# vLAR-group/NVFi

Hardware: AMD Instinct MI355X
Metric: training rays/sec (fwd+bwd incl. PDE loss), 'bat' scene (higher is better)
Workload: dtype f32; 1 GPU; bat.yaml + velocity field + PDE divergence loss (configs[2]): 199^3 grid, K=16, 128 samples/ray, 2 renders x 2048 rays + PDE on 262144 collocation points + plane regularisers + Adam, per GPU; pde_points_per_gpu=262144, samples_per_ray=128, parallelism=ray-sharded x1, driver=fused, launch=eager launches, field=stationary (optimiser steps a shadow copy)

## Files before the change

nvfi_amd/csrc/vel_x6w.hip:

```cpp
#include <stdlib.h>
#include <utility>
#include "common.h"
#include "vel.h"
#include "pde.h"
#include "engine16.h"
#include "x6.h"

typedef unsigned u32x4w __attribute__((ext_vector_type(4)));
typedef const b8_t __attribute__((address_space(1))) * x6w_gptr;
#define X6W_ENTRIES 136
#define X6W_RING 8
#define X6W_OB_H8 (8 * 3 * 64)
#define X6W_LDS_BYTES ((6 * 128 + 4 * 2 * 16 * 8) * 4 + 4 * X6W_OB_H8 * 16)

#ifdef X6W_TIMING
__device__ unsigned long long x6w_ts[32];
#define X6W_STAMP(c, k) do { if ((c).stamp) x6w_ts[k] = __builtin_amdgcn_s_memtime(); } while (0)
#else
#define X6W_STAMP(c, k) do { } while (0)
#endif
#if defined(X6W_BUFLD)
typedef unsigned u32x4b __attribute__((ext_vector_type(4)));
#define X6W_OPAQUE(c) asm volatile("" : "+s"((c).so))
#define X6W_LD(c, P, E) __builtin_bit_cast(b8_t, __builtin_amdgcn_raw_buffer_load_b128((c).R##P, (int)(c).vo + (E) * 1024, (c).so, 0))
#define X6W_PTR(img, lane) ((x6w_gptr)(img))
#else
#define X6W_OPAQUE(c) asm volatile("" : "+v"((c).W1), "+v"((c).W2), "+v"((c).W3))
#define X6W_LD(c, P, E) ((c).P[(E) * 64])
#define X6W_PTR(img, lane) ((x6w_gptr)((img) + (lane)))
#endif
struct X6W {
    int stamp;
    unsigned vo;
#ifdef X6W_BUFLD
    __amdgpu_buffer_rsrc_t RW1, RW2, RW3; int so;
#endif
    x6w_gptr W1, W2, W3;
    const float* lb;
    const float4* w5l;
    b8_t* ob;
    float* zp;
    int lane, h;
};

template <int... Is, class F> __device__ __forceinline__ void x6w_for(std::integer_sequence<int, Is...>, F f) { (f(std::integral_constant<int, Is>{}), ...); }

struct X6WEpi {
    float rr[16];
    unsigned pk[3][8];
    float p[6];
    float4 wa, wb;
    float out[6];
    float* zst;
};
__device__ __forceinline__ float x6w_add_halves(float p) {
    const auto r = __builtin_amdgcn_permlane32_swap(__float_as_uint(p), __float_as_uint(p), false, false);
    return __uint_as_float(r[0]) + __uint_as_float(r[1]);
}
template <int U, bool LAST, int STASH = 0, bool PX4 = false>
__device__ __forceinline__ void x6w_micro(const X6W& c, float (&v)[16], X6WEpi& e, int m2) {
    if constexpr (STASH && U < 32 && (U & 1) == 0) {
        if constexpr (PX4) {
            if constexpr ((U & 7) == 0) {
                const f32x4s q = {v[U >> 1], v[(U >> 1) + 1], v[(U >> 1) + 2], v[(U >> 1) + 3]};
                __builtin_nontemporal_store(q, reinterpret_cast<f32x4s*>(e.zst - c.lane) + c.lane + (U >> 3) * 64);
            }
        } else STASH_ST(e.zst[(U >> 1) * REGF], v[U >> 1]);
    }
#ifndef X6W_PROBE_NO_SILU
    if constexpr (U < 32) {
        constexpr int r = U >> 1;
        if constexpr ((U & 1) == 0) e.rr[r] = __builtin_amdgcn_exp2f(-1.44269504088896341f * v[r]);
        else e.rr[r] = __builtin_amdgcn_rcpf(1.f + e.rr[r]);
    }
    if constexpr (U >= 2 && U <= 32 && (U & 1) == 0) { constexpr int r = (U - 2) >> 1; v[r] = v[r] * e.rr[r]; }
#endif
    if constexpr (LAST) {
        const float4* wl = c.w5l + ((m2 >> 1) * 2 + c.h) * 32;
        if constexpr (U == 0) {
#pragma unroll
            for (int o = 0; o < 6; ++o) e.p[o] = 0.f;
        }
        if constexpr (U == 1) e.wa = wl[0];
        if constexpr (U == 2) e.wb = wl[1];
        x6w_for(std::make_integer_sequence<int, 48>{}, [&](auto Gc) {
            constexpr int g = decltype(Gc)::value, r = g / 3, j = g % 3;
            if constexpr (3 + g - g / 8 == U) {
                if constexpr (j == 0) { e.p[0] = __builtin_fmaf(v[r], e.wa.x, e.p[0]); e.p[1] = __builtin_fmaf(v[r], e.wa.y, e.p[1]); }
                if constexpr (j == 1) {
                    e.p[2] = __builtin_fmaf(v[r], e.wa.z, e.p[2]); e.p[3] = __builtin_fmaf(v[r], e.wa.w, e.p[3]);
                    if constexpr (r < 15) e.wa = wl[2 * (r + 1)];
                }
                if constexpr (j == 2) {
                    e.p[4] = __builtin_fmaf(v[r], e.wb.x, e.p[4]); e.p[5] = __builtin_fmaf(v[r], e.wb.y, e.p[5]);
                    if constexpr (r < 15) e.wb = wl[2 * (r + 1) + 1];
                }
            }
        });
        if constexpr (U == 46) {
#pragma unroll
            for (int o = 0; o < 3; ++o) e.p[o] = x6w_add_halves(e.p[o]);
        }
        if constexpr (U == 47) {
#pragma unroll
            for (int o = 3; o < 6; ++o) e.p[o] = x6w_add_halves(e.p[o]);
#pragma unroll
            for (int o = 0; o < 6; ++o) e.out[o] += e.p[o];
        }
    } else {
        if constexpr (U >= 5 && U <= 36) {
            constexpr int p = (U - 5) >> 2, part = (U - 5) & 3;
#ifdef X6W_PROBE_NO_SPLIT
            if constexpr (part == 0) {
                e.pk[0][p] = __builtin_amdgcn_perm(__float_as_uint(v[2 * p + 1]), __float_as_uint(v[2 * p]), 0x07060302u);
                e.pk[1][p] = e.pk[0][p]; e.pk[2][p] = e.pk[0][p];
            }
#else
            if constexpr (part == 0) {
                const unsigned ua = __float_as_uint(v[2 * p]), ub = __float_as_uint(v[2 * p + 1]);
                e.pk[0][p] = __builtin_amdgcn_perm(ub, ua, 0x07060302u);
                e.rr[2 * p] = v[2 * p] - __uint_as_float(ua & 0xffff0000u);
            } else if constexpr (part == 1) {
                e.rr[2 * p + 1] = v[2 * p + 1] - __uint_as_float(__float_as_uint(v[2 * p + 1]) & 0xffff0000u);
            } else if constexpr (part == 2) {
                const unsigned va = __float_as_uint(e.rr[2 * p]), vb = __float_as_uint(e.rr[2 * p + 1]);
                e.pk[1][p] = __builtin_amdgcn_perm(vb, va, 0x07060302u);
                e.rr[2 * p] = e.rr[2 * p] - __uint_as_float(va & 0xffff0000u);
            } else {
                const float sb = e.rr[2 * p + 1] - __uint_as_float(__float_as_uint(e.rr[2 * p + 1]) & 0xffff0000u);
                e.pk[2][p] = __builtin_amdgcn_perm(__float_as_uint(sb), __float_as_uint(e.rr[2 * p]), 0x07060302u);
            }
#endif
        }
        if constexpr (U == 22 || U == 37) {
            constexpr int k = U == 22 ? 0 : 1;
#pragma unroll
            for (int term = 0; term < 3; ++term) {
                const u32x4w q = {e.pk[term][4 * k], e.pk[term][4 * k + 1], e.pk[term][4 * k + 2], e.pk[term][4 * k + 3]};
                c.ob[((size_t)(m2 + k) * 3 + term) * 64] = __builtin_bit_cast(b8_t, q);
            }
        }
    }
}
template <int U0, int N, bool LAST, int STASH = 0, bool PX4 = false>
__device__ __forceinline__ void x6w_micros(const X6W& c, float (&v)[16], X6WEpi& e, int m2) {
    x6w_for(std::make_integer_sequence<int, N>{}, [&](auto Uc) {
        constexpr int U = U0 + decltype(Uc)::value;
        if constexpr (U < (LAST ? 48 : 38)) x6w_micro<U, LAST, STASH, PX4>(c, v, e, m2);
    });
}
__device__ __forceinline__ void x6w_load_in(const X6W& c, b8_t (&in)[8][3], int s) {
    in[s][0] = c.ob[((size_t)s * 3 + 0) * 64]; in[s][1] = c.ob[((size_t)s * 3 + 1) * 64]; in[s][2] = c.ob[((size_t)s * 3 + 2) * 64];
}

template <int J, bool FIRST>
__device__ __forceinline__ void x6w_mfma(const b8_t& A1, const b8_t& A2, const b8_t& A3, const b8_t (&B)[3], f32x16& a0, f32x16& a1) {
    const f32x16 zero = {0.f, 0.f, 0.f, 0.f, 0.f, 0.f, 0.f, 0.f, 0.f, 0.f, 0.f, 0.f, 0.f, 0.f, 0.f, 0.f};
    if constexpr (J == 0) a0 = MFMA16B(A1, B[0], a0);
    else if constexpr (J == 1) a1 = MFMA16B(A1, B[1], FIRST ? zero : a1);
    else if constexpr (J == 2) a1 = MFMA16B(A2, B[1], a1);
    else if constexpr (J == 3) a1 = MFMA16B(A2, B[0], a1);
    else if constexpr (J == 4) a1 = MFMA16B(A1, B[2], a1);
    else a1 = MFMA16B(A3, B[0], a1);
}

template <int E0, int KIND, int LROW, bool HAVE_PE, bool PE_LAST, int STASH = 0>
__device__ __forceinline__ void x6w_tile(X6W& c, b8_t (&A1)[X6W_RING], b8_t (&A2)[X6W_RING], b8_t (&A3)[X6W_RING], const b8_t (&X0)[2][3], b8_t (&in)[8][3],
                                         float (&pv)[16], X6WEpi& e, int pm2, float (&nv)[16], f32x16& bias) {
    constexpr int NS = KIND == 0 ? 2 : 8;
    f32x16 a0 = bias, a1;
    x6w_for(std::make_integer_sequence<int, NS * 6>{}, [&](auto Ic) {
        constexpr int I = decltype(Ic)::value, s = I / 6, j = I % 6, en = E0 + s;
        if constexpr (KIND == 0) x6w_mfma<j, s == 0>(A1[en % X6W_RING], A2[en % X6W_RING], A3[en % X6W_RING], X0[s], a0, a1);
        else x6w_mfma<j, s == 0>(A1[en % X6W_RING], A2[en % X6W_RING], A3[en % X6W_RING], in[s], a0, a1);
        __builtin_amdgcn_sched_barrier(0);
        if constexpr (j == 5 && en + X6W_RING - 1 < X6W_ENTRIES + X6W_RING - 1) {
            constexpr int x = en + X6W_RING - 1;
            if constexpr ((x & 3) == 0) {
#ifndef X6W_PROBE_SAME_ENTRIES
#ifdef X6W_BUFLD
                c.so += (x == X6W_ENTRIES) ? -(X6W_ENTRIES / 4 - 1) * 4096 : 4096;
#else
                constexpr int adv = (x == X6W_ENTRIES) ? -(X6W_ENTRIES / 4 - 1) * 256 : 256;
                c.W1 += adv; c.W2 += adv; c.W3 += adv;
#endif
#endif
                X6W_OPAQUE(c);
            }
#if defined(X6W_PROBE_QUARTER_LOADS)
            if constexpr ((x & 3) == 0) { A1[x % X6W_RING] = X6W_LD(c, W1, 0); A2[x % X6W_RING] = X6W_LD(c, W2, 0); A3[x % X6W_RING] = X6W_LD(c, W3, 0); }
#elif defined(X6W_PROBE_LDS_A)
            A1[x % X6W_RING] = c.ob[((x & 7) * 3 + 0) * 64]; A2[x % X6W_RING] = c.ob[((x & 7) * 3 + 1) * 64]; A3[x % X6W_RING] = c.ob[((x & 7) * 3 + 2) * 64];
#else
            A1[x % X6W_RING] = X6W_LD(c, W1, x & 3); A2[x % X6W_RING] = X6W_LD(c, W2, x & 3); A3[x % X6W_RING] = X6W_LD(c, W3, x & 3);
#endif
        }
#ifndef X6W_PROBE_NO_EPILOGUE
        if constexpr (HAVE_PE) {
            if constexpr (KIND == 0) {
                if constexpr (I < 2) x6w_micros<4 * I, 4, PE_LAST, STASH, (STASH == 2 && LROW >= 32 && LROW - 32 < 512)>(c, pv, e, pm2);
                else x6w_micros<8 + 3 * (I - 2), 3, PE_LAST, STASH, (STASH == 2 && LROW >= 32 && LROW - 32 < 512)>(c, pv, e, pm2);
            } else if constexpr (KIND == 1) {
                if constexpr (I < 8) x6w_micros<2 * I, 2, PE_LAST, STASH, (STASH == 2 && LROW >= 32 && LROW - 32 < 512)>(c, pv, e, pm2);
                else if constexpr (I < 30) x6w_micros<I + 8, 1, PE_LAST, STASH, (STASH == 2 && LROW >= 32 && LROW - 32 < 512)>(c, pv, e, pm2);
            } else if constexpr (I < (PE_LAST ? 48 : 38)) x6w_micros<I, 1, PE_LAST, STASH, (STASH == 2 && LROW >= 32 && LROW - 32 < 512)>(c, pv, e, pm2);
        }
#endif
        if constexpr (KIND == 1 && I == 30) { x6w_load_in(c, in, 6); x6w_load_in(c, in, 7); }
        if constexpr (I == 1 && LROW + 32 < 640) {
#pragma unroll
            for (int r = 0; r < 16; ++r) bias[r] = c.lb[LROW + 32 + (r & 3) + 8 * (r >> 2) + 4 * c.h];
        }
        if constexpr (KIND == 3) {
            if constexpr (j == 5 && s < 4) x6w_load_in(c, in, s);
            if constexpr (I == 40) { x6w_load_in(c, in, 4); x6w_load_in(c, in, 5); }
        }
        __builtin_amdgcn_sched_barrier(0);
    });
#pragma unroll
    for (int r = 0; r < 16; ++r) nv[r] = a1[r] + a0[r];
    if constexpr (STASH) {
        if constexpr (KIND == 4) {
#pragma unroll
            for (int r = 0; r < 16; ++r) STASH_ST(c.zp[r * REGF], nv[r]);
        } else e.zst = c.zp;
        c.zp += 16 * REGF;
        asm volatile("" : "+v"(c.zp));
    }
    X6W_STAMP(c, E0 < 8 ? 1 + E0 / 2 : 5 + (E0 - 8) / 8);
    __builtin_amdgcn_sched_barrier(0);
}

struct X6WRing { b8_t A1[X6W_RING], A2[X6W_RING], A3[X6W_RING]; };
__device__ __forceinline__ void x6w_prime(const X6W& c0, X6WRing& R) {
    X6W c = c0;
    X6W_OPAQUE(c);
#pragma unroll
    for (int en = 0; en < X6W_RING - 1; ++en) {
#ifdef X6W_BUFLD
        if (en == 4) c.so += 4096;
#else
        if (en == 4) { c.W1 += 256; c.W2 += 256; c.W3 += 256; }
#endif
        R.A1[en] = X6W_LD(c, W1, en & 3); R.A2[en] = X6W_LD(c, W2, en & 3); R.A3[en] = X6W_LD(c, W3, en & 3);
    }
}
template <int STASH = 0>
__device__ __forceinline__ void velnet_x6w(const X6W& c0, X6WRing& R, const float4& q, float (&out6)[6], float* zst = nullptr, float* x0st = nullptr) {
    X6W c = c0;
    X6W_STAMP(c, 0);
    c.zp = STASH ? zst + c0.lane : nullptr;
    X6W_OPAQUE(c);
    b8_t X0[2][3], in[8][3];
    b8_t (&A1)[X6W_RING] = R.A1, (&A2)[X6W_RING] = R.A2, (&A3)[X6W_RING] = R.A3;
    X6WEpi e;
    float va[16], vb[16];
    {
        float x0[16];
#ifdef X6W_PROBE_NO_ENC
#pragma unroll
        for (int k = 0; k < 16; ++k) x0[k] = q.x + (float)k * q.y;
#else
        vel_encode_slots(q, c.h, x0);
#endif
        if (STASH) stash_store<16>(x0st, c.lane, x0);
#pragma unroll
        for (int k = 0; k < 2; ++k) {
            unsigned p1[4], p2[4], p3[4];
#pragma unroll
            for (int j = 0; j < 4; ++j) {
                const float xa = x0[8 * k + 2 * j], xb = x0[8 * k + 2 * j + 1];
                const unsigned ua = __float_as_uint(xa), ub = __float_as_uint(xb);
                p1[j] = __builtin_amdgcn_perm(ub, ua, 0x07060302u);
                const float ra = xa - __uint_as_float(ua & 0xffff0000u), rb = xb - __uint_as_float(ub & 0xffff0000u);
                const unsigned wa = __float_as_uint(ra), wb = __float_as_uint(rb);
                p2[j] = __builtin_amdgcn_perm(wb, wa, 0x07060302u);
                const float sa = ra - __uint_as_float(wa & 0xffff0000u), sb = rb - __uint_as_float(wb & 0xffff0000u);
                p3[j] = __builtin_amdgcn_perm(__float_as_uint(sb), __float_as_uint(sa), 0x07060302u);
            }
            const u32x4w q1 = {p1[0], p1[1], p1[2], p1[3]}, q2 = {p2[0], p2[1], p2[2], p2[3]}, q3 = {p3[0], p3[1], p3[2], p3[3]};
            X0[k][0] = __builtin_bit_cast(b8_t, q1); X0[k][1] = __builtin_bit_cast(b8_t, q2); X0[k][2] = __builtin_bit_cast(b8_t, q3);
        }
    }
#ifdef X6W_BUFLD
    c.so += 4096;
#else
    c.W1 += 256; c.W2 += 256; c.W3 += 256;
#endif
    f32x16 bias;
#pragma unroll
    for (int r = 0; r < 16; ++r) bias[r] = c.lb[(r & 3) + 8 * (r >> 2) + 4 * c.h];
#pragma unroll
    for (int o = 0; o < 6; ++o) e.out[o] = c.lb[128 * 5 + o];
    x6w_tile<0, 0, 0, false, false, STASH>(c, A1, A2, A3, X0, in, va, e, 0, va, bias);
    x6w_tile<2, 0, 32, true, false, STASH>(c, A1, A2, A3, X0, in, va, e, 0, vb, bias);
    x6w_tile<4, 0, 64, true, false, STASH>(c, A1, A2, A3, X0, in, vb, e, 2, va, bias);
    x6w_tile<6, 0, 96, true, false, STASH>(c, A1, A2, A3, X0, in, va, e, 4, vb, bias);
#pragma unroll
    for (int s = 0; s < 6; ++s) x6w_load_in(c, in, s);
    x6w_tile<8, 1, 128, true, false, STASH>(c, A1, A2, A3, X0, in, vb, e, 6, va, bias);
    x6w_tile<16, 2, 160, true, false, STASH>(c, A1, A2, A3, X0, in, va, e, 0, vb, bias);
    x6w_tile<24, 2, 192, true, false, STASH>(c, A1, A2, A3, X0, in, vb, e, 2, va, bias);
    x6w_tile<32, 3, 224, true, false, STASH>(c, A1, A2, A3, X0, in, va, e, 4, vb, bias);
    x6w_tile<40, 1, 256, true, false, STASH>(c, A1, A2, A3, X0, in, vb, e, 6, va, bias);
    x6w_tile<48, 2, 288, true, false, STASH>(c, A1, A2, A3, X0, in, va, e, 0, vb, bias);
    x6w_tile<56, 2, 320, true, false, STASH>(c, A1, A2, A3, X0, in, vb, e, 2, va, bias);
    x6w_tile<64, 3, 352, true, false, STASH>(c, A1, A2, A3, X0, in, va, e, 4, vb, bias);
    x6w_tile<72, 1, 384, true, false, STASH>(c, A1, A2, A3, X0, in, vb, e, 6, va, bias);
    x6w_tile<80, 2, 416, true, false, STASH>(c, A1, A2, A3, X0, in, va, e, 0, vb, bias);
    x6w_tile<88, 2, 448, true, false, STASH>(c, A1, A2, A3, X0, in, vb, e, 2, va, bias);
    x6w_tile<96, 3, 480, true, false, STASH>(c, A1, A2, A3, X0, in, va, e, 4, vb, bias);
    x6w_tile<104, 1, 512, true, false, STASH>(c, A1, A2, A3, X0, in, vb, e, 6, va, bias);
    x6w_tile<112, 2, 544, true, true, STASH>(c, A1, A2, A3, X0, in, va, e, 0, vb, bias);
    x6w_tile<120, 2, 576, true, true, STASH>(c, A1, A2, A3, X0, in, vb, e, 2, va, bias);
    x6w_tile<128, 4, 608, true, true, STASH>(c, A1, A2, A3, X0, in, va, e, 4, vb, bias);
#ifdef X6W_PROBE_NO_OUT
#pragma unroll
    for (int o = 0; o < 6; ++o) out6[o] = e.out[o];
    out6[0] += vb[0]; out6[1] += vb[5];
    return;
#endif
    {
        float p[6] = {0.f, 0.f, 0.f, 0.f, 0.f, 0.f};
        const float4* wl = c.w5l + (3 * 2 + c.h) * 32;
#pragma unroll
        for (int r = 0; r < 16; ++r) {
            const float4 wa = wl[2 * r], wb = wl[2 * r + 1];
            const float av = act_f<1>(vb[r]);
            p[0] = __builtin_fmaf(av, wa.x, p[0]); p[1] = __builtin_fmaf(av, wa.y, p[1]); p[2] = __builtin_fmaf(av, wa.z, p[2]);
            p[3] = __builtin_fmaf(av, wa.w, p[3]); p[4] = __builtin_fmaf(av, wb.x, p[4]); p[5] = __builtin_fmaf(av, wb.y, p[5]);
        }
#pragma unroll
        for (int o = 0; o < 6; ++o) out6[o] = e.out[o] + x6w_add_halves(p[o]);
    }
    X6W_STAMP(c, 21);
}

__global__ __launch_bounds__(WG_THREADS, 1) void k_rk2_x6w(X6Args a) {
    extern __shared__ __attribute__((aligned(16))) float lds[];
    float* lb = lds;
    float* w5f = lb + 6 * 128;
    b8_t* obase = reinterpret_cast<b8_t*>(w5f + 4 * 2 * 16 * 8);
    const int lane = threadIdx.x & 63, h = lane >> 5;
    const int wv = __builtin_amdgcn_readfirstlane(threadIdx.x >> 6);
    const int count = a.count ? *a.count : (int)a.n_direct;
    if ((int)blockIdx.x * 4 * TILE >= count) return;
    for (int k = threadIdx.x; k < 6 * 128; k += WG_THREADS) lb[k] = (k & 127) < (k < 640 ? 128 : 6) ? a.f.vb[k >> 7][k & 127] : 0.f;
    for (int k = threadIdx.x; k < 4 * 2 * 16 * 8; k += WG_THREADS) {
        const int o = k & 7, r = (k >> 3) & 15, hh = (k >> 7) & 1, ww = k >> 8;
        w5f[k] = o < 6 ? a.f.vW[5][o * 128 + 32 * ww + (r & 3) + 8 * (r >> 2) + 4 * hh] : 0.f;
    }
    __syncthreads();
    const int tile = blockIdx.x * 4 + wv;
    if (tile * TILE >= count) return;
    const int i = tile * TILE + (lane & 31);
    const bool active = i < count;
    const int n = active ? (a.list ? a.list[i] : i) : 0;
    const float4 q0 = active ? a.xw[n] : zero4();
    float x = q0.x, y = q0.y, z = q0.z;
    const float zw = q0.w;
    const int ti = a.pt_by_list ? n : i;
    float tcur = active ? a.pt_t[ti] : 0.f;
    float off = active ? tcur - a.pt_base[ti] : 0.f;
    X6W c; c.stamp = 0;
    const b8_t* img = reinterpret_cast<const b8_t*>(a.img);
    c.W1 = X6W_PTR(img, lane); c.W2 = X6W_PTR(img + X6_H8, lane); c.W3 = X6W_PTR(img + 2 * X6_H8, lane); c.vo = (unsigned)lane * 16u;
#ifdef X6W_BUFLD
    c.so = 0;
    c.RW1 = __builtin_amdgcn_make_buffer_rsrc(const_cast<b8_t*>(img), 0, 0x7fffffff, 0x00020000);
    c.RW2 = __builtin_amdgcn_make_buffer_rsrc(const_cast<b8_t*>(img + X6_H8), 0, 0x7fffffff, 0x00020000);
    c.RW3 = __builtin_amdgcn_make_buffer_rsrc(const_cast<b8_t*>(img + 2 * X6_H8), 0, 0x7fffffff, 0x00020000);
#endif
    c.lb = lb; c.w5l = reinterpret_cast<const float4*>(w5f); c.ob = obase + (size_t)wv * X6W_OB_H8 + lane; c.lane = lane; c.h = h;
    X6WRing ring;
    x6w_prime(c, ring);
#pragma unroll 1
    for (int s = 0; s < a.max_steps; ++s) {
        const bool live = active && fabsf(off) > 0.f;
        const float dt = rk2_point_dt(off, a.dt_max);
        if (!__any(live)) break;
        const float hdt = 0.5f * dt;
        float px = x, py = y, pz = z;
        float o6[6];
#pragma unroll 1
        for (int ev = 0; ev < 2; ++ev) {
            const float4 q = make_float4(px, py, pz, ev ? tcur - hdt : tcur);
#ifdef X6W_TIMING
            c.stamp = (blockIdx.x == 700 && wv == 1 && s == 2 && ev == 0) ? 1 : 0;
#endif
            velnet_x6w(c, ring, q, o6);
            if (ev == 0) {
                float v1[3];
                vel_from_w(o6, x, y, z, v1);
                if (gated_out(a.f, x, y, z)) { v1[0] = v1[1] = v1[2] = 0.f; }
                px = x - hdt * v1[0]; py = y - hdt * v1[1]; pz = z - hdt * v1[2];
            }
        }
        float v2[3];
        vel_from_w(o6, px, py, pz, v2);
        if (gated_out(a.f, px, py, pz)) { v2[0] = v2[1] = v2[2] = 0.f; }
        const float nx = x - dt * v2[0], ny = y - dt * v2[1], nz = z - dt * v2[2];
        const bool rej = a.f.gate_sur && gated_out(a.f, nx, ny, nz);
        if (live && !rej) { x = nx; y = ny; z = nz; }
        if (live) { off = off - dt; tcur = tcur - dt; }
    }
#ifdef X6W_TIMING
    if (blockIdx.x == 700 && wv == 1 && lane == 0) {
        printf("[x6w timing] tiles (layer 0: 4, layers 1-4: 4 each), then the last row tile's sums:");
        for (int k = 1; k <= 21; ++k) printf(" %llu", x6w_ts[k] - x6w_ts[k - 1]);
        printf(" | total %llu\n", x6w_ts[21] - x6w_ts[0]);
    }
#endif
    if (active && h == 0) {
        if (a.xout3) { float* o = a.xout3 + 3 * (size_t)n; o[0] = x; o[1] = y; o[2] = z; }
        else a.xw[n] = make_float4(x, y, z, zw);
    }
}

template <int STASH>
__global__ __launch_bounds__(WG_THREADS, 1) void k_rk2_x6w_uni(X6UniArgs a) {
    extern __shared__ __attribute__((aligned(16))) float lds[];
    float* lb = lds;
    float* w5f = lb + 6 * 128;
    b8_t* obase = reinterpret_cast<b8_t*>(w5f + 4 * 2 * 16 * 8);
    const Rk2Args& ra = a.r;
    const int lane = threadIdx.x & 63, h = lane >> 5;
    const int wv = __builtin_amdgcn_readfirstlane(threadIdx.x >> 6);
    const int count = *ra.count;
    if ((int)blockIdx.x * WG_SAMPLES >= count) return;
    for (int k = threadIdx.x; k < 6 * 128; k += WG_THREADS) lb[k] = (k & 127) < (k < 640 ? 128 : 6) ? ra.f.vb[k >> 7][k & 127] : 0.f;
    for (int k = threadIdx.x; k < 4 * 2 * 16 * 8; k += WG_THREADS) {
        const int o = k & 7, r = (k >> 3) & 15, hh = (k >> 7) & 1, ww = k >> 8;
        w5f[k] = o < 6 ? ra.f.vW[5][o * 128 + 32 * ww + (r & 3) + 8 * (r >> 2) + 4 * hh] : 0.f;
    }
    __syncthreads();
    const size_t tile = (size_t)blockIdx.x * 4 + wv;
    if (!STASH && (int)(tile * TILE) >= count) return;
    const int idx = (int)tile * TILE + (lane & 31);
    const bool active = idx < count;
    const int n = active ? ra.list[idx] : 0;
    const float4 q0 = active ? ra.xw[n] : zero4();
    float x = q0.x, y = q0.y, z = q0.z;
    const float zw = q0.w;
    X6W c; c.stamp = 0;
    const b8_t* img = reinterpret_cast<const b8_t*>(a.img);
    c.W1 = X6W_PTR(img, lane); c.W2 = X6W_PTR(img + X6_H8, lane); c.W3 = X6W_PTR(img + 2 * X6_H8, lane); c.vo = (unsigned)lane * 16u;
#ifdef X6W_BUFLD
    c.so = 0;
    c.RW1 = __builtin_amdgcn_make_buffer_rsrc(const_cast<b8_t*>(img), 0, 0x7fffffff, 0x00020000);
    c.RW2 = __builtin_amdgcn_make_buffer_rsrc(const_cast<b8_t*>(img + X6_H8), 0, 0x7fffffff, 0x00020000);
    c.RW3 = __builtin_amdgcn_make_buffer_rsrc(const_cast<b8_t*>(img + 2 * X6_H8), 0, 0x7fffffff, 0x00020000);
#endif
    c.lb = lb; c.w5l = reinterpret_cast<const float4*>(w5f); c.ob = obase + (size_t)wv * X6W_OB_H8 + lane; c.lane = lane; c.h = h; c.zp = nullptr;
    const int nsteps = ra.sched ? __float_as_int(ra.sched[2]) : ra.nsteps;
    X6WRing ring;
    x6w_prime(c, ring);
#pragma unroll 1
    for (int s = 0; s < nsteps; ++s) {
        const float dt = RK_DT(ra, s), tcur = RK_TC(ra, s), hdt = 0.5f * dt;
        float px = x, py = y, pz = z;
        float o6[6], w1[6];
        bool g1 = false;
#pragma unroll 1
        for (int ev = 0; ev < 2; ++ev) {
            const size_t e = (size_t)(2 * s + ev) * ra.cap_tiles + tile;
            const float4 q = make_float4(px, py, pz, ev ? tcur - hdt : tcur);
            velnet_x6w<STASH>(c, ring, q, o6, STASH ? ra.zst + e * (VEL_Z_REGS * REGF) : nullptr, STASH ? ra.x0st + e * (VEL_X0_REGS * REGF) : nullptr);
            if (ev == 0) {
                float v1[3];
#pragma unroll
                for (int k = 0; k < 6; ++k) w1[k] = o6[k];
                vel_from_w(w1, x, y, z, v1);
                g1 = gated_out(ra.f, x, y, z);
                if (g1) { v1[0] = v1[1] = v1[2] = 0.f; }
                px = x - hdt * v1[0]; py = y - hdt * v1[1]; pz = z - hdt * v1[2];
            }
        }
        float v2[3];
        vel_from_w(o6, px, py, pz, v2);
        const bool g2 = gated_out(ra.f, px, py, pz);
        if (g2) { v2[0] = v2[1] = v2[2] = 0.f; }
        const float nx = x - dt * v2[0], ny = y - dt * v2[1], nz = z - dt * v2[2];
        const bool rej = ra.f.gate_sur && gated_out(ra.f, nx, ny, nz);
        if (STASH && active && h == 0) {
            float* rc = ra.rec + (size_t)s * RK_NF * ra.cap + idx;
            rc[0 * ra.cap] = x; rc[1 * ra.cap] = y; rc[2 * ra.cap] = z;
            rc[3 * ra.cap] = px; rc[4 * ra.cap] = py; rc[5 * ra.cap] = pz;
#pragma unroll
            for (int k = 0; k < 6; ++k) { rc[(6 + k) * ra.cap] = w1[k]; rc[(12 + k) * ra.cap] = o6[k]; }
            rc[18 * ra.cap] = __int_as_float((g1 ? 1 : 0) | (g2 ? 2 : 0) | (rej ? 4 : 0));
        }
        if (active && !rej) { x = nx; y = ny; z = nz; }
    }
    if (active && h == 0) ra.xw[n] = make_float4(x, y, z, zw);
}

int launch_rk2_x6w_uni(const X6UniArgs& a, int64_t cap_samples, bool stash, hipStream_t st) {
    const int64_t groups = (cap_samples + WG_SAMPLES - 1) / WG_SAMPLES;
    if (groups <= 0) return 0;
    static DeviceOnce once;
    if (once.lds(X6W_LDS_BYTES, k_rk2_x6w_uni<2>, k_rk2_x6w_uni<1>, k_rk2_x6w_uni<0>)) return 1;
    if (stash && a.r.z_x4) hipLaunchKernelGGL(k_rk2_x6w_uni<2>, dim3((unsigned)groups), dim3(WG_THREADS), X6W_LDS_BYTES, st, a);
    else if (stash) hipLaunchKernelGGL(k_rk2_x6w_uni<1>, dim3((unsigned)groups), dim3(WG_THREADS), X6W_LDS_BYTES, st, a);
    else hipLaunchKernelGGL(k_rk2_x6w_uni<0>, dim3((unsigned)groups), dim3(WG_THREADS), X6W_LDS_BYTES, st, a);
    LAUNCHCK();
    return 0;
}

int launch_rk2_x6w(const X6Args& a, int64_t cap_points, hipStream_t st) {
    const int64_t tiles = (cap_points + TILE - 1) / TILE;
    if (tiles <= 0) return 0;
    static DeviceOnce once;
    if (once.lds(X6W_LDS_BYTES, k_rk2_x6w)) return 1;
    hipLaunchKernelGGL(k_rk2_x6w, dim3((unsigned)((tiles + 3) / 4)), dim3(WG_THREADS), X6W_LDS_BYTES, st, a);
    LAUNCHCK();
    return 0;
}
```

Measured before the change: 1.105 million rays/s.

## Process two point tiles per wave in RK2 velocity MLP to share weight loads

Adds a new RK2 kernel in which each wave advects two 32-point tiles at once. It interleaves their MFMA chains so that each weight fragment loaded from global memory is reused for both tiles. The weight ring is shortened to 4 entries and the LDS staging buffer is split per tile to make room for the doubled activation state. The new kernel is the default unless the switch selects the old path. It raises register pressure and halves the number of waves covering the points, which can hurt latency hiding. The shared LDS staging and context setup are factored into helpers.

```diff
diff --git a/nvfi_amd/csrc/vel_x6w.hip b/nvfi_amd/csrc/vel_x6w.hip
--- a/nvfi_amd/csrc/vel_x6w.hip
+++ b/nvfi_amd/csrc/vel_x6w.hip
@@ -336,23 +336,28 @@
     X6W_STAMP(c, 21);
 }
 
-__global__ __launch_bounds__(WG_THREADS, 1) void k_rk2_x6w(X6Args a) {
-    extern __shared__ __attribute__((aligned(16))) float lds[];
-    float* lb = lds;
-    float* w5f = lb + 6 * 128;
-    b8_t* obase = reinterpret_cast<b8_t*>(w5f + 4 * 2 * 16 * 8);
-    const int lane = threadIdx.x & 63, h = lane >> 5;
-    const int wv = __builtin_amdgcn_readfirstlane(threadIdx.x >> 6);
-    const int count = a.count ? *a.count : (int)a.n_direct;
-    if ((int)blockIdx.x * 4 * TILE >= count) return;
-    for (int k = threadIdx.x; k < 6 * 128; k += WG_THREADS) lb[k] = (k & 127) < (k < 640 ? 128 : 6) ? a.f.vb[k >> 7][k & 127] : 0.f;
+__device__ __forceinline__ void x6w_stage_lds(const nvfi_field_desc& f, float* lb, float* w5f) {
+    for (int k = threadIdx.x; k < 6 * 128; k += WG_THREADS) lb[k] = (k & 127) < (k < 640 ? 128 : 6) ? f.vb[k >> 7][k & 127] : 0.f;
     for (int k = threadIdx.x; k < 4 * 2 * 16 * 8; k += WG_THREADS) {
         const int o = k & 7, r = (k >> 3) & 15, hh = (k >> 7) & 1, ww = k >> 8;
-        w5f[k] = o < 6 ? a.f.vW[5][o * 128 + 32 * ww + (r & 3) + 8 * (r >> 2) + 4 * hh] : 0.f;
-    }
-    __syncthreads();
-    const int tile = blockIdx.x * 4 + wv;
-    if (tile * TILE >= count) return;
+        w5f[k] = o < 6 ? f.vW[5][o * 128 + 32 * ww + (r & 3) + 8 * (r >> 2) + 4 * hh] : 0.f;
+    }
+}
+__device__ __forceinline__ void x6w_context(X6W& c, const void* image, float* lb, float* w5f, b8_t* ob, int lane) {
+    c.stamp = 0;
+    const b8_t* img = reinterpret_cast<const b8_t*>(image);
+    c.W1 = X6W_PTR(img, lane); c.W2 = X6W_PTR(img + X6_H8, lane); c.W3 = X6W_PTR(img + 2 * X6_H8, lane); c.vo = (unsigned)lane * 16u;
+#ifdef X6W_BUFLD
+    c.so = 0;
+    c.RW1 = __builtin_amdgcn_make_buffer_rsrc(const_cast<b8_t*>(img), 0, 0x7fffffff, 0x00020000);
+    c.RW2 = __builtin_amdgcn_make_buffer_rsrc(const_cast<b8_t*>(img + X6_H8), 0, 0x7fffffff, 0x00020000);
+    c.RW3 = __builtin_amdgcn_make_buffer_rsrc(const_cast<b8_t*>(img + 2 * X6_H8), 0, 0x7fffffff, 0x00020000);
+#endif
+    c.lb = lb; c.w5l = reinterpret_cast<const float4*>(w5f); c.ob = ob + lane; c.lane = lane; c.h = lane >> 5;
+}
+
+__device__ __forceinline__ void x6w_rk2_one(const X6Args& a, X6W& c, int tile, int count, int wv) {
+    const int lane = c.lane, h = c.h;
     const int i = tile * TILE + (lane & 31);
     const bool active = i < count;
     const int n = active ? (a.list ? a.list[i] : i) : 0;
@@ -362,16 +367,6 @@
     const int ti = a.pt_by_list ? n : i;
     float tcur = active ? a.pt_t[ti] : 0.f;
     float off = active ? tcur - a.pt_base[ti] : 0.f;
-    X6W c; c.stamp = 0;
-    const b8_t* img = reinterpret_cast<const b8_t*>(a.img);
-    c.W1 = X6W_PTR(img, lane); c.W2 = X6W_PTR(img + X6_H8, lane); c.W3 = X6W_PTR(img + 2 * X6_H8, lane); c.vo = (unsigned)lane * 16u;
-#ifdef X6W_BUFLD
-    c.so = 0;
-    c.RW1 = __builtin_amdgcn_make_buffer_rsrc(const_cast<b8_t*>(img), 0, 0x7fffffff, 0x00020000);
-    c.RW2 = __builtin_amdgcn_make_buffer_rsrc(const_cast<b8_t*>(img + X6_H8), 0, 0x7fffffff, 0x00020000);
-    c.RW3 = __builtin_amdgcn_make_buffer_rsrc(const_cast<b8_t*>(img + 2 * X6_H8), 0, 0x7fffffff, 0x00020000);
-#endif
-    c.lb = lb; c.w5l = reinterpret_cast<const float4*>(w5f); c.ob = obase + (size_t)wv * X6W_OB_H8 + lane; c.lane = lane; c.h = h;
     X6WRing ring;
     x6w_prime(c, ring);
 #pragma unroll 1
@@ -386,7 +381,7 @@
         for (int ev = 0; ev < 2; ++ev) {
             const float4 q = make_float4(px, py, pz, ev ? tcur - hdt : tcur);
 #ifdef X6W_TIMING
-            c.stamp = (blockIdx.x == 700 && wv == 1 && s == 2 && ev == 0) ? 1 : 0;
+            c.stamp = (blockIdx.x == 16 && wv == 1 && s == 1 && ev == 0) ? 1 : 0;
 #endif
             velnet_x6w(c, ring, q, o6);
             if (ev == 0) {
@@ -405,7 +400,7 @@
         if (live) { off = off - dt; tcur = tcur - dt; }
     }
 #ifdef X6W_TIMING
-    if (blockIdx.x == 700 && wv == 1 && lane == 0) {
+    if (blockIdx.x == 16 && wv == 1 && lane == 0) {
         printf("[x6w timing] tiles (layer 0: 4, layers 1-4: 4 each), then the last row tile's sums:");
         for (int k = 1; k <= 21; ++k) printf(" %llu", x6w_ts[k] - x6w_ts[k - 1]);
         printf(" | total %llu\n", x6w_ts[21] - x6w_ts[0]);
@@ -415,6 +410,238 @@
         if (a.xout3) { float* o = a.xout3 + 3 * (size_t)n; o[0] = x; o[1] = y; o[2] = z; }
         else a.xw[n] = make_float4(x, y, z, zw);
     }
+}
+__global__ __launch_bounds__(WG_THREADS, 1) void k_rk2_x6w(X6Args a) {
+    extern __shared__ __attribute__((aligned(16))) float lds[];
+    float* lb = lds;
+    float* w5f = lb + 6 * 128;
+    b8_t* obase = reinterpret_cast<b8_t*>(w5f + 4 * 2 * 16 * 8);
+    const int lane = threadIdx.x & 63;
+    const int wv = __builtin_amdgcn_readfirstlane(threadIdx.x >> 6);
+    const int count = a.count ? *a.count : (int)a.n_direct;
+    if ((int)blockIdx.x * 4 * TILE >= count) return;
+    x6w_stage_lds(a.f, lb, w5f);
+    __syncthreads();
+    const int tile = blockIdx.x * 4 + wv;
+    if (tile * TILE >= count) return;
+    X6W c;
+    x6w_context(c, a.img, lb, w5f, obase + (size_t)wv * X6W_OB_H8, lane);
+    x6w_rk2_one(a, c, tile, count, wv);
+}
+
+#define X6W2_RING 4
+#define X6W2_OB_H8 (6 * 3 * 64)
+#define X6W2_LDS_BYTES ((6 * 128 + 4 * 2 * 16 * 8) * 4 + 4 * 2 * X6W2_OB_H8 * 16)
+struct X6WRing2 { b8_t A1[X6W2_RING], A2[X6W2_RING], A3[X6W2_RING]; };
+__device__ __forceinline__ void x6w_prime2(const X6W& c0, X6WRing2& R) {
+    X6W c = c0;
+    X6W_OPAQUE(c);
+#pragma unroll
+    for (int en = 0; en < X6W2_RING - 1; ++en) { R.A1[en] = X6W_LD(c, W1, en); R.A2[en] = X6W_LD(c, W2, en); R.A3[en] = X6W_LD(c, W3, en); }
+}
+__device__ __forceinline__ void x6w_load_in2(const X6W& c, b8_t (&in)[8][3], int s, int slot) {
+    in[s][0] = c.ob[((size_t)slot * 3 + 0) * 64]; in[s][1] = c.ob[((size_t)slot * 3 + 1) * 64]; in[s][2] = c.ob[((size_t)slot * 3 + 2) * 64];
+}
+template <int E0, int KIND, int LROW, bool HAVE_PE, bool PE_LAST>
+__device__ __forceinline__ void x6w_tile2(X6W& c, const X6W& c1, X6WRing2& R, const b8_t (&X0)[2][2][3], b8_t (&in)[2][8][3],
+                                          float (&pv)[2][16], X6WEpi (&e)[2], int pm2, float (&nv)[2][16], f32x16& bias, int lrow = LROW) {
+    constexpr int NS = KIND == 0 ? 2 : 8;
+    f32x16 a0[2] = {bias, bias}, a1[2];
+    x6w_for(std::make_integer_sequence<int, NS * 12>{}, [&](auto Ic) {
+        constexpr int II = decltype(Ic)::value, s = II / 12, t = (II % 12) / 6, j = II % 6, I = 6 * s + j, en = E0 + s, sl = en % X6W2_RING;
+        const X6W& ct = t ? c1 : c;
+        if constexpr (KIND == 0) x6w_mfma<j, s == 0>(R.A1[sl], R.A2[sl], R.A3[sl], X0[t][s], a0[t], a1[t]);
+        else x6w_mfma<j, s == 0>(R.A1[sl], R.A2[sl], R.A3[sl], in[t][s], a0[t], a1[t]);
+        __builtin_amdgcn_sched_barrier(0);
+        if constexpr (t == 0 && j == 5) {
+            constexpr int x = en + X6W2_RING - 1;
+            if constexpr ((x & 3) == 0) {
+#ifdef X6W_BUFLD
+                c.so += (x == X6W_ENTRIES) ? -(X6W_ENTRIES / 4 - 1) * 4096 : 4096;
+#else
+                constexpr int adv = (x == X6W_ENTRIES) ? -(X6W_ENTRIES / 4 - 1) * 256 : 256;
+                c.W1 += adv; c.W2 += adv; c.W3 += adv;
+#endif
+                X6W_OPAQUE(c);
+            }
+            R.A1[x % X6W2_RING] = X6W_LD(c, W1, x & 3); R.A2[x % X6W2_RING] = X6W_LD(c, W2, x & 3); R.A3[x % X6W2_RING] = X6W_LD(c, W3, x & 3);
+        }
+        if constexpr (HAVE_PE) {
+            if constexpr (KIND == 0) {
+                if constexpr (I < 2) x6w_micros<4 * I, 4, PE_LAST>(ct, pv[t], e[t], pm2);
+                else x6w_micros<8 + 3 * (I - 2), 3, PE_LAST>(ct, pv[t], e[t], pm2);
+            } else if constexpr (KIND == 1) {
+                if constexpr (I < 8) x6w_micros<2 * I, 2, PE_LAST>(ct, pv[t], e[t], pm2);
+                else if constexpr (I < 30) x6w_micros<I + 8, 1, PE_LAST>(ct, pv[t], e[t], pm2);
+            } else if constexpr (I < (PE_LAST ? 48 : 38)) x6w_micros<I, 1, PE_LAST>(ct, pv[t], e[t], pm2);
+        }
+        if constexpr (KIND == 1 && I == 30) { x6w_load_in2(ct, in[t], 6, 0); x6w_load_in2(ct, in[t], 7, 1); }
+        if constexpr (II == 7 && LROW + 32 < 640) {
+#pragma unroll
+            for (int r = 0; r < 16; ++r) bias[r] = c.lb[lrow + 32 + (r & 3) + 8 * (r >> 2) + 4 * c.h];
+        }
+        if constexpr (KIND == 3) {
+            if constexpr (j == 5 && s < 4) x6w_load_in2(ct, in[t], s, s);
+            if constexpr (I == 40) { x6w_load_in2(ct, in[t], 4, 4); x6w_load_in2(ct, in[t], 5, 5); }
+        }
+        __builtin_amdgcn_sched_barrier(0);
+    });
+#pragma unroll
+    for (int t = 0; t < 2; ++t) {
+#pragma unroll
+        for (int r = 0; r < 16; ++r) nv[t][r] = a1[t][r] + a0[t][r];
+    }
+    __builtin_amdgcn_sched_barrier(0);
+}
+__device__ __forceinline__ void velnet_x6w2(const X6W& c0, const X6W& c1, X6WRing2& R, const float4 (&q)[2], float (&out6)[2][6]) {
+    X6W c = c0;
+    X6W_STAMP(c, 0);
+    X6W_OPAQUE(c);
+    b8_t X0[2][2][3], in[2][8][3];
+    X6WEpi e[2];
+    float va[2][16], vb[2][16];
+#pragma unroll
+    for (int t = 0; t < 2; ++t) {
+        float x0[16];
+        vel_encode_slots(q[t], c.h, x0);
+#pragma unroll
+        for (int k = 0; k < 2; ++k) x6_split8(x0 + 8 * k, X0[t][k][0], X0[t][k][1], X0[t][k][2]);
+    }
+    f32x16 bias;
+#pragma unroll
+    for (int r = 0; r < 16; ++r) bias[r] = c.lb[(r & 3) + 8 * (r >> 2) + 4 * c.h];
+#pragma unroll
+    for (int t = 0; t < 2; ++t) {
+#pragma unroll
+        for (int o = 0; o < 6; ++o) e[t].out[o] = c.lb[128 * 5 + o];
+    }
+    x6w_tile2<0, 0, 0, false, false>(c, c1, R, X0, in, va, e, 0, va, bias);
+    x6w_tile2<2, 0, 32, true, false>(c, c1, R, X0, in, va, e, 0, vb, bias);
+    x6w_tile2<4, 0, 64, true, false>(c, c1, R, X0, in, vb, e, 2, va, bias);
+    x6w_tile2<6, 0, 96, true, false>(c, c1, R, X0, in, va, e, 4, vb, bias);
+    X6W_STAMP(c, 1);
+#pragma unroll
+    for (int s = 0; s < 6; ++s) { x6w_load_in2(c, in[0], s, s); x6w_load_in2(c1, in[1], s, s); }
+#pragma unroll 1
+    for (int lrow = 128; lrow < 512; lrow += 128) {
+        x6w_tile2<8, 1, 128, true, false>(c, c1, R, X0, in, vb, e, 0, va, bias, lrow);
+        x6w_tile2<16, 2, 160, true, false>(c, c1, R, X0, in, va, e, 0, vb, bias, lrow + 32);
+        x6w_tile2<24, 2, 192, true, false>(c, c1, R, X0, in, vb, e, 2, va, bias, lrow + 64);
+        x6w_tile2<32, 3, 224, true, false>(c, c1, R, X0, in, va, e, 4, vb, bias, lrow + 96);
+        X6W_STAMP(c, 1 + lrow / 128);
+    }
+    x6w_tile2<104, 1, 512, true, false>(c, c1, R, X0, in, vb, e, 0, va, bias);
+    x6w_tile2<112, 2, 544, true, true>(c, c1, R, X0, in, va, e, 0, vb, bias);
+    x6w_tile2<120, 2, 576, true, true>(c, c1, R, X0, in, vb, e, 2, va, bias);
+    x6w_tile2<128, 4, 608, true, true>(c, c1, R, X0, in, va, e, 4, vb, bias);
+    X6W_STAMP(c, 5);
+    const float4* wl = c.w5l + (3 * 2 + c.h) * 32;
+#pragma unroll
+    for (int t = 0; t < 2; ++t) {
+        float p[6] = {0.f, 0.f, 0.f, 0.f, 0.f, 0.f};
+#pragma unroll
+        for (int r = 0; r < 16; ++r) {
+            const float4 wa = wl[2 * r], wb = wl[2 * r + 1];
+            const float av = act_f<1>(vb[t][r]);
+            p[0] = __builtin_fmaf(av, wa.x, p[0]); p[1] = __builtin_fmaf(av, wa.y, p[1]); p[2] = __builtin_fmaf(av, wa.z, p[2]);
+            p[3] = __builtin_fmaf(av, wa.w, p[3]); p[4] = __builtin_fmaf(av, wb.x, p[4]); p[5] = __builtin_fmaf(av, wb.y, p[5]);
+        }
+#pragma unroll
+        for (int o = 0; o < 6; ++o) out6[t][o] = e[t].out[o] + x6w_add_halves(p[o]);
+    }
+    X6W_STAMP(c, 6);
+}
+__device__ __forceinline__ void x6w_rk2_pair(const X6Args& a, X6W& c, const X6W& c1, int tile0, int count, int wv) {
+    const int lane = c.lane, h = c.h;
+    bool active[2];
+    int n[2];
+    float x[2], y[2], z[2], zw[2], tcur[2], off[2];
+#pragma unroll
+    for (int t = 0; t < 2; ++t) {
+        const int i = (tile0 + t) * TILE + (lane & 31);
+        active[t] = i < count;
+        n[t] = active[t] ? (a.list ? a.list[i] : i) : 0;
+        const float4 q0 = active[t] ? a.xw[n[t]] : zero4();
+        x[t] = q0.x; y[t] = q0.y; z[t] = q0.z; zw[t] = q0.w;
+        const int ti = a.pt_by_list ? n[t] : i;
+        tcur[t] = active[t] ? a.pt_t[ti] : 0.f;
+        off[t] = active[t] ? tcur[t] - a.pt_base[ti] : 0.f;
+    }
+    X6WRing2 ring;
+    x6w_prime2(c, ring);
+#pragma unroll 1
+    for (int s = 0; s < a.max_steps; ++s) {
+        bool live[2];
+        float dt[2], hdt[2], px[2], py[2], pz[2];
+#pragma unroll
+        for (int t = 0; t < 2; ++t) { live[t] = active[t] && fabsf(off[t]) > 0.f; dt[t] = rk2_point_dt(off[t], a.dt_max); }
+        if (!__any(live[0] || live[1])) break;
+#pragma unroll
+        for (int t = 0; t < 2; ++t) { hdt[t] = 0.5f * dt[t]; px[t] = x[t]; py[t] = y[t]; pz[t] = z[t]; }
+        float o6[2][6];
+#pragma unroll 1
+        for (int ev = 0; ev < 2; ++ev) {
+            const float4 q[2] = {make_float4(px[0], py[0], pz[0], ev ? tcur[0] - hdt[0] : tcur[0]), make_float4(px[1], py[1], pz[1], ev ? tcur[1] - hdt[1] : tcur[1])};
+#ifdef X6W_TIMING
+            c.stamp = (blockIdx.x == 8 && wv == 1 && s == 1 && ev == 0) ? 1 : 0;
+#endif
+            velnet_x6w2(c, c1, ring, q, o6);
+            if (ev == 0) {
+#pragma unroll
+                for (int t = 0; t < 2; ++t) {
+                    float v1[3];
+                    vel_from_w(o6[t], x[t], y[t], z[t], v1);
+                    if (gated_out(a.f, x[t], y[t], z[t])) { v1[0] = v1[1] = v1[2] = 0.f; }
+                    px[t] = x[t] - hdt[t] * v1[0]; py[t] = y[t] - hdt[t] * v1[1]; pz[t] = z[t] - hdt[t] * v1[2];
+                }
+            }
+        }
+#pragma unroll
+        for (int t = 0; t < 2; ++t) {
+            float v2[3];
+            vel_from_w(o6[t], px[t], py[t], pz[t], v2);
+            if (gated_out(a.f, px[t], py[t], pz[t])) { v2[0] = v2[1] = v2[2] = 0.f; }
+            const float nx = x[t] - dt[t] * v2[0], ny = y[t] - dt[t] * v2[1], nz = z[t] - dt[t] * v2[2];
+            const bool rej = a.f.gate_sur && gated_out(a.f, nx, ny, nz);
+            if (live[t] && !rej) { x[t] = nx; y[t] = ny; z[t] = nz; }
+            if (live[t]) { off[t] = off[t] - dt[t]; tcur[t] = tcur[t] - dt[t]; }
+        }
+    }
+#ifdef X6W_TIMING
+    if (blockIdx.x == 8 && wv == 1 && lane == 0) {
+        printf("[x6w2 timing] layer 0, layers 1-4, the last row tile's sums:");
+        for (int k = 1; k <= 6; ++k) printf(" %llu", x6w_ts[k] - x6w_ts[k - 1]);
+        printf(" | total %llu\n", x6w_ts[6] - x6w_ts[0]);
+    }
+#endif
+    if (h == 0) {
+#pragma unroll
+        for (int t = 0; t < 2; ++t) {
+            if (!active[t]) continue;
+            if (a.xout3) { float* o = a.xout3 + 3 * (size_t)n[t]; o[0] = x[t]; o[1] = y[t]; o[2] = z[t]; }
+            else a.xw[n[t]] = make_float4(x[t], y[t], z[t], zw[t]);
+        }
+    }
+}
+__global__ __launch_bounds__(WG_THREADS, 1) void k_rk2_x6w2(X6Args a) {
+    extern __shared__ __attribute__((aligned(16))) float lds[];
+    float* lb = lds;
+    float* w5f = lb + 6 * 128;
+    b8_t* obase = reinterpret_cast<b8_t*>(w5f + 4 * 2 * 16 * 8);
+    const int lane = threadIdx.x & 63;
+    const int wv = __builtin_amdgcn_readfirstlane(threadIdx.x >> 6);
+    const int count = a.count ? *a.count : (int)a.n_direct;
+    if ((int)blockIdx.x * 8 * TILE >= count) return;
+    x6w_stage_lds(a.f, lb, w5f);
+    __syncthreads();
+    const int tile0 = (blockIdx.x * 4 + wv) * 2;
+    if (tile0 * TILE >= count) return;
+    X6W c;
+    x6w_context(c, a.img, lb, w5f, obase + (size_t)wv * 2 * X6W2_OB_H8, lane);
+    if ((tile0 + 1) * TILE >= count) { x6w_rk2_one(a, c, tile0, count, wv); return; }
+    X6W c1 = c;
+    c1.ob = c.ob + X6W2_OB_H8;
+    x6w_rk2_pair(a, c, c1, tile0, count, wv);
 }
 
 template <int STASH>
@@ -510,6 +737,13 @@
 int launch_rk2_x6w(const X6Args& a, int64_t cap_points, hipStream_t st) {
     const int64_t tiles = (cap_points + TILE - 1) / TILE;
     if (tiles <= 0) return 0;
+    if (sw(NVFI_X6W) != 2) {
+        static DeviceOnce once2;
+        if (once2.lds(X6W2_LDS_BYTES, k_rk2_x6w2)) return 1;
+        hipLaunchKernelGGL(k_rk2_x6w2, dim3((unsigned)((tiles + 7) / 8)), dim3(WG_THREADS), X6W2_LDS_BYTES, st, a);
+        LAUNCHCK();
+        return 0;
+    }
     static DeviceOnce once;
     if (once.lds(X6W_LDS_BYTES, k_rk2_x6w)) return 1;
     hipLaunchKernelGGL(k_rk2_x6w, dim3((unsigned)((tiles + 3) / 4)), dim3(WG_THREADS), X6W_LDS_BYTES, st, a);
```

Result: no change. 1.112 million rays/s, median of 4 (+0.7%).
